# Entscheider/depthhead

Measured on AMD Instinct MI355X. Metric: depth frames/sec (640x480, 10-tree forest), higher is better.
Workload: dtype u32/f64

## Files before the change

### depthhead_amd/csrc/dh_api.hip

```cpp
#include "dh_runtime.h"
#include "dh_render.h"
#include "dh_runtime_track.h"

extern "C" const char *dh_last_error(void) { return dh_err_get_(); }
extern "C" int dh_version(void) { return DH_VERSION; }

static int forest_create_(const dh_forest_desc *d, dh_forest **out) { return dh_forest_build_(d, out); }

static int forest_destroy_(dh_forest *f) {
    delete f;
    return DH_OK;
}

static int forest_info_(const dh_forest *f, uint32_t *n_trees, uint32_t *n_nodes, uint32_t *n_leaves, uint32_t *max_depth) {
    if (!f) return fail(DH_EINVAL, "dh_forest_info: NULL forest");
    if (n_trees) *n_trees = (uint32_t)f->roots.size();
    if (n_nodes) *n_nodes = (uint32_t)f->nodes.size();
    if (n_leaves) *n_leaves = (uint32_t)f->leaf_prob.size();
    if (max_depth) *max_depth = f->max_depth;
    return DH_OK;
}

static int patch_grid_(const dh_params *p, int w, int h, int *nx, int *ny) {
    if (!p || !nx || !ny) return fail(DH_EINVAL, "dh_patch_grid: NULL argument");
// ... 538 lines not shown
    BoxArgs ba{};
    ba.frames = L.q.frames; ba.zeros = L.p->zeros.get(); ba.n_frames = L.n; ba.w = L.w; ba.h = L.h; ba.rw = L.p->f_rw; ba.rh = L.p->f_rh;
    ba.tile_flags = L.tile_flags; ba.tiles_x = g.tiles_x; ba.tiles_y = g.tiles_y; ba.gen = L.gen; ba.tpx = L.tpx; ba.tpy = L.tpy; ba.tbw = L.tw; ba.tbh = L.th;
    if (L.o.zero_fold) { ba.zero_ptr = ws.counters.get(); ba.zero_lo = (uint32_t)ws.lay.zero_lo; ba.zero_hi = (uint32_t)ws.lay.zero_hi; ba.zero_end = (uint32_t)ws.lay.zero_words; }
    ba.out = L.box; ba.plane = g.box_plane; ba.rows = g.box_rows; ba.lg = g.swz_log2; ba.ow = g.box_ow; ba.parts = g.box_parts;
    ba.ring = L.bp.ring; ba.oh = L.bp.oh; ba.bands = L.bp.bands; ba.blocks_per_frame = L.bp.blocks_per_frame;
    ba.blk_shift = ws.blk_shift; ba.mask_blocks = L.bp.mask_blocks; ba.blk_mask = L.blk_mask;
    if (L.use_list && ws.shifts.on) ba.list_count = L.tl_count;
    { Range r(L.o.profile, "dh:boxsum"); HIP_TRY(dh_launch_boxsum(ba, L.s)); }
    return DH_OK;
}
static int enqueue_tile_list(const Launch &L) {
    const Workspace &ws = L.ws; const Geom &g = L.g;
    Range r(L.o.profile, "dh:tile_list");
    if (!ws.shifts.on) { HIP_TRY(dh_launch_tile_list(L.tile_flags, L.gen, L.n, g.tiles_x * g.tiles_y, L.tl_list, L.tl_count, (uint32_t)ws.tile_list_stride, L.s)); return DH_OK; }
    TileShiftArgs sa{};
    sa.n_frames = L.n; sa.blk_shift = ws.blk_shift; sa.mask_blocks = L.bp.mask_blocks; sa.parts = g.box_parts; sa.blk_mask = L.blk_mask; sa.ow4 = g.box_ow / 4; sa.nc = g.box_parts * sa.ow4;
    sa.tiles_x = g.tiles_x; sa.tiles_y = g.tiles_y; sa.step = L.step; sa.tpx = L.tpx; sa.tpy = L.tpy; sa.tbw = L.tw; sa.tbh = L.th;
    sa.sx0 = ws.shifts.sx0; sa.sy0 = ws.shifts.sy0; sa.gx = ws.shifts.gx; sa.nsx = ws.shifts.nsx; sa.nsy = ws.shifts.nsy;
    sa.list = L.tl_list; sa.count = L.tl_count; sa.stride = (uint32_t)ws.tile_list_stride; sa.shift_out = ws.tile_shift.get() + L.f0;
    HIP_TRY(dh_launch_tile_shift(sa, L.s));
    return DH_OK;
}
static int enqueue_traverse(const Launch &L, bool *gated) {
    dh_predictor *p = L.p;
    const Workspace &ws = L.ws; const Geom &g = L.g;
    TraverseArgs ta{};
    ta.frames = L.q.frames; ta.n_frames = L.n; ta.w = L.w; ta.h = L.h;
    ta.step = L.step; ta.sw = (int)p->params.subimage_width; ta.sh = (int)p->params.subimage_height;
    ta.nx = g.nx; ta.ny = g.ny; ta.px = g.px; ta.py = g.py; ta.tiles_x = g.tiles_x; ta.tiles_y = g.tiles_y;
    ta.ss_max = g.ss_max; ta.ss_row = g.ss_row; ta.swz_log2 = g.swz_log2; ta.swz_q = g.swz_q;
    ta.uniform = g.uniform ? 1 : 0; ta.rw = p->f_rw; ta.rh = p->f_rh; ta.area = (uint32_t)(p->f_rw * p->f_rh);
    ta.nodes_u = p->nodes_u.get(); ta.nodes_a = p->absorb_ok ? p->nodes_a.get() : nullptr; ta.walk_lb = (p->n_nodes + p->n_amb) << 4; ta.amb_list = p->amb_list.get();
    ta.top_tab = p->top_tab.get(); ta.top_levels = g.top_levels; ta.nodes_g = p->knobs.no_general_int ? nullptr : p->nodes_g.get();
    ta.box = L.box; ta.box_plane = g.box_plane; ta.box_rows = g.box_rows; ta.tile_flags = L.tile_flags; ta.gen = L.gen;
#ifdef DH_PROFILING_KNOBS
    ta.stop_phase = p->knobs.trav_stop;
    if (p->knobs.trav_stamps)
        TRY(next_stamps(p->trav_stamps, 8, &ta.dbg_stamps, [](const unsigned long long *hst) {
            fprintf(stderr, "[k_traverse cycles/phase summed over the workgroups that reach it] region=%llu gate=%llu walks=%llu gated tail=%llu\n", hst[0], hst[1], hst[2], hst[3]);
        }));
#endif
    ta.f = p->dev; set_windows(ta, ws, L.f0, p->n_trees);
    *gated = !L.o.traverse_only && !L.o.leaf_out && !L.o.flags_out && dh_tile_gate_(g, ws.cap_frames, p->absorb_ok, p->n_trees, p->debug, p->knobs);
    if (*gated) { ta.tile_gate = 1; ta.win_total = ws.win_total(L.f0); }
    if (!L.o.traverse_only) p->ws.last_gated = *gated;
    ta.dbg_flags = L.dbg_flags; ta.dbg_leaf = L.o.leaf_out ? L.o.leaf_out : p->debug ? ws.dbg_leaf.get() + (size_t)L.f0 * g.npatch * p->n_trees : nullptr;
    if (L.use_list) { ta.tile_list = L.tl_list; ta.tile_list_count = L.tl_count; ta.tile_list_stride = (uint32_t)ws.tile_list_stride; }
    { Range r(L.o.profile, "dh:traverse"); HIP_TRY(dh_launch_traverse(ta, g.lds, L.s)); }
    return DH_OK;
}
static int enqueue_emit(const Launch &L, bool gated) {
    const Geom &g = L.g;
    EmitArgs ea{};
    ea.frames = L.q.frames; ea.n_frames = L.n; ea.w = L.w; ea.h = L.h;
    ea.step = L.step; ea.lw = L.lw; ea.lh = L.lh; ea.nx = g.nx; ea.npatch = g.npatch; ea.px = g.px; ea.py = g.py; ea.tiles = g.tiles_x * g.tiles_y;
    memcpy(ea.kinv, L.kinv, sizeof ea.kinv);
    ea.cams = L.cams; ea.f = L.p->dev; set_windows(ea, L.ws, L.f0, L.p->n_trees);
    if (gated) { ea.pre_gated = 1; ea.win_total = L.ws.win_total(L.f0); }
    set_hits(ea, L.ws, L.f0);
    ea.leaf_hits = L.q.heads ? nullptr : L.leaf_hits;
    ea.gen = L.gen; ea.dbg_flags = L.dbg_flags;
    if (L.q.support || L.q.heads) ea.hit_win = L.ws.hit_win.get() + L.hoff;
#ifdef DH_PROFILING_KNOBS
    ea.stop = L.p->knobs.emit_stop;
#endif
    { Range r(L.o.profile, "dh:emit"); HIP_TRY(dh_launch_emit(ea, L.s)); }
    return DH_OK;
}
static int enqueue_vote(const Launch &L) {
    const CamSel &cs = L.q.cams;
    VoteArgs va{};
    va.n_frames = L.n; va.w = L.w; va.h = L.h;
    va.cell_fast = !L.p->knobs.vote_exact && (!cs.c || cs.all_cell_fast(L.n, L.w, L.h)) ? 1 : 0;
    memcpy(va.k, L.K, sizeof va.k);
    va.cams = L.cams; va.cams_pin = cs.c && cs.all_pin(L.n) ? 1 : 0; va.f = L.p->dev;
    set_hits(va, L.ws, L.f0);
    va.pos_grid = L.pos_grid; va.rot_grid = L.rot_grid; va.leaf_hits = L.q.heads ? nullptr : L.leaf_hits;
#ifdef DH_PROFILING_KNOBS
    va.stop = L.p->knobs.vote_stop;
#endif
    { Range r(L.o.profile, "dh:vote"); HIP_TRY(dh_launch_vote(va, L.s)); }
    return DH_OK;
}
static ClusterArgs cluster_args(const Launch &L) {
    ClusterArgs ca{};
    ca.frames = L.q.frames; ca.n_frames = L.n; ca.w = L.w; ca.h = L.h;
    memcpy(ca.kinv, L.kinv, sizeof ca.kinv);
    ca.cams = L.cams; ca.f = L.p->dev; set_hits(ca, L.ws, L.f0);
    ca.pos_grid = L.pos_grid; ca.kern_r2 = L.p->kern_r2.get(); ca.iterations = L.p->params.meanshift_iterations;
    return ca;
}
static int enqueue_cluster(const Launch &L) {
    dh_predictor *p = L.p; const Workspace &ws = L.ws;
    ClusterArgs ca = cluster_args(L);
// ... 50 lines not shown
    SupportArgs sa{};
    sa.n_frames = L.n; sa.nx = L.g.nx; sa.step = L.step; sa.lw = L.lw; sa.lh = L.lh;
    sa.radius = L.q.radius; sa.poses = L.q.out; sa.out = L.q.support;
    sa.hits = ws.hits.get() + L.hoff; sa.hit_box = ws.hit_box.get() + L.hoff; sa.hit_win = ws.hit_win.get() + L.hoff;
    sa.hit_count = L.hit_count; sa.hits_cap = ws.hits_cap; sa.off4 = L.p->dev.off4;
    sa.acc = ws.sup_acc.get() + L.f0; sa.bits = ws.sup_bits.get() + (size_t)L.f0 * ws.sup_words; sa.bit_words = ws.sup_words;
    { Range r(L.o.profile, "dh:support"); HIP_TRY(dh_launch_support(sa, L.s)); }
    return DH_OK;
}

static int enqueue_range(dh_predictor *p, const BatchReq &sl, int f0, int n, hipStream_t s, const EnqueueOpts &o) {
    Launch L{p, sl.at(f0), f0, n, s, o};
    if (L.q.cams.c) memcpy(L.kinv, L.q.cams.c->host[L.q.cams.c0].kinv, sizeof L.kinv);
    else dh_mat3_inv_f32_(L.K, L.kinv);
    if (L.use_list) p->ws.list_chunks = std::max(p->ws.list_chunks, o.chunk + 1);
    const bool windows = L.g.npatch > 0;
    char batch_name[48];
    snprintf(batch_name, sizeof batch_name, "dh:batch n=%d %dx%d", n, L.w, L.h);
    Range batch_range(o.profile, batch_name);
    if (o.profile) HIP_TRY(hipEventRecord(p->ev[0], s));
    if (windows) TRY(enqueue_flags(L));
    if (L.use_list) TRY(enqueue_tile_list(L));
    if (o.profile) HIP_TRY(hipEventRecord(p->ev[4], s));
    bool gated = false;
    if (windows) TRY(enqueue_traverse(L, &gated));
    if (o.profile) HIP_TRY(hipEventRecord(p->ev[5], s));
    if (windows && !o.traverse_only) TRY(enqueue_emit(L, gated));
    if (o.profile) HIP_TRY(hipEventRecord(p->ev[1], s));
    if (o.traverse_only) return DH_OK;
    TRY(enqueue_vote(L));
    if (o.profile) HIP_TRY(hipEventRecord(p->ev[2], s));
    if (L.q.heads) TRY(enqueue_heads(L));
    else {
        TRY(enqueue_cluster(L));
        if (L.q.support) TRY(enqueue_support(L));
    }
    if (o.profile) { HIP_TRY(hipEventRecord(p->ev[3], s)); p->ev_valid = true; }
    return DH_OK;
}

static int max_resident_frames(const dh_predictor *p) { return p->knobs.max_resident; }

static int support_reserve(dh_predictor *p) {
    Workspace &ws = p->ws;
    if (ws.sup) return DH_OK;
    const size_t cap = (size_t)ws.cap_frames;
    ws.sup_words = (uint32_t)((std::max(ws.geom.npatch, 1) + 31) / 32);
    TRY(ws.hit_win.alloc(cap * ws.hits_cap));
    TRY(ws.sup_acc.alloc(cap));
    TRY(ws.sup_bits.alloc(cap * ws.sup_words));
    TRY(ws.sup.alloc(cap));
    if (hipMemsetAsync(ws.sup_acc.get(), 0, cap * sizeof(SupAcc), p->own_stream) != hipSuccess ||
        hipMemsetAsync(ws.sup_bits.get(), 0, cap * ws.sup_words * sizeof(uint32_t), p->own_stream) != hipSuccess ||
// ... 1011 lines not shown
        const Workspace &ws = p->ws;
        const Geom &g = ws.geom;
        const size_t bytes = (size_t)p->last_n * 4;
        if (g.npatch <= 0) { memset(out, 0, bytes); return DH_OK; }
        if (ws.last_gated) { HIP_TRY(hipMemcpy(out, ws.win_total(0), bytes, hipMemcpyDeviceToHost)); return DH_OK; }
        Buf<uint32_t> tot;
        TRY(tot.alloc(p->last_n));
        HIP_TRY(hipMemset(tot.get(), 0, bytes));
        EmitArgs ea{};
        ea.n_frames = p->last_n; ea.px = g.px; ea.py = g.py; ea.tiles = g.tiles_x * g.tiles_y; ea.f = p->dev;
        set_windows(ea, ws, 0, p->n_trees);
        HIP_TRY(dh_launch_window_totals(ea, tot.get(), nullptr));
        HIP_TRY(hipDeviceSynchronize());
        HIP_TRY(hipMemcpy(out, tot.get(), bytes, hipMemcpyDeviceToHost));
        return DH_OK;
    });
}
static int debug_geometry_(dh_predictor *p, int32_t out[10]) {
    if (!p || !out) return fail(DH_EINVAL, "NULL argument");
    if (p->ws.cap_frames == 0) return fail(DH_ESTATE, "no workspace yet (dh_predictor_reserve or a batch)");
    const Geom &g = p->ws.geom;
    const bool walk_tab = g.uniform && p->absorb_ok;
    const bool tile_gate = dh_tile_gate_(g, p->ws.cap_frames, p->absorb_ok, p->n_trees, p->debug, p->knobs);
    const int32_t v[10] = {(g.uniform ? 1 : 0) | (walk_tab ? 1 << 8 : 0) | (tile_gate ? 1 << 9 : 0) | (walk_tab ? g.top_levels << 16 : 0), g.px, g.py, g.tiles_x, g.tiles_y, g.swz_log2, g.swz_q, g.ss_row, p->f_rw, p->f_rh};
    memcpy(out, v, sizeof v);
    return DH_OK;
}
static int debug_tile_shifts_(dh_predictor *p, int32_t *shifts, uint32_t counts[8]) {
    return with_taps(p, false, [&]() -> int {
        const Workspace &ws = p->ws;
        if (!shifts || !counts) return fail(DH_EINVAL, "NULL output");
        if (ws.list_chunks == 0) return fail(DH_ESTATE, "the last batch ran without tile lists");
        std::vector<uint32_t> sh((size_t)p->last_n, 0u);
        if (ws.tile_shift) HIP_TRY(hipMemcpy(sh.data(), ws.tile_shift.get(), sh.size() * 4, hipMemcpyDeviceToHost));
        for (int f = 0; f < p->last_n; ++f) { shifts[2 * f] = (int32_t)(sh[f] & 0xffffu); shifts[2 * f + 1] = (int32_t)(sh[f] >> 16); }
        for (int x = 0; x < 8; ++x) counts[x] = 0;
        for (int c = 0; c < ws.list_chunks; ++c) {
            uint32_t cc[8];
            HIP_TRY(hipMemcpy(cc, ws.list_ptr(c) + 16 * ws.tile_list_stride, sizeof cc, hipMemcpyDeviceToHost));
            for (int x = 0; x < 8; ++x) counts[x] += cc[x];
        }
        return DH_OK;
    });
}
static int debug_guesses_(dh_predictor *p, int32_t *out) {
    return with_taps(p, true, [&]() -> int {
        if (!out) return fail(DH_EINVAL, "NULL output");
// ... 126 lines not shown
```

### depthhead_amd/csrc/dh_host.cpp

```cpp
#include "dh_host.h"

#include <limits.h>
#include <math.h>
#include <stdarg.h>
#include <stdio.h>
#include <stdlib.h>
#include <string.h>

#include <algorithm>
#include <cmath>
#include <atomic>
#include <string>
#include <thread>
#include <utility>

static thread_local char g_err[512] = "";

int dh_fail_(int code, const char *fmt, ...) {
    va_list ap;
    va_start(ap, fmt);
    vsnprintf(g_err, sizeof g_err, fmt, ap);
    va_end(ap);
    return code;
}
// ... 139 lines not shown
}

Knobs dh_read_knobs_() {
    Knobs k;
    auto geti = [](const char *name, int dflt) { const char *e = getenv(name); return e ? atoi(e) : dflt; };
    k.force_general = getenv("DH_FORCE_GENERAL") != nullptr;
    k.no_leaf_hist = getenv("DH_NO_LEAF_HIST") != nullptr;
    k.box_no_ring = getenv("DH_BOX_NO_RING") != nullptr;
    k.leaf_hist_max = (uint32_t)std::max(0, geti("DH_LEAF_HIST_MAX", 16384));
    k.lds_budget_kb = std::max(0, geti("DH_LDS_BUDGET_KB", 0));
    if (const char *e = getenv("DH_TILE")) {
        if (sscanf(e, "%d,%d", &k.tile_x, &k.tile_y) != 2 || k.tile_x < 1 || k.tile_y < 1) k.tile_x = k.tile_y = 0;
    }
    k.box_band = std::max(1, geti("DH_BOX_BAND", 64));
    k.box_bands = std::max(0, geti("DH_BOX_BANDS", 0));
    k.max_resident = std::max(1, geti("DH_MAX_RESIDENT_FRAMES", 512));
    k.chunks = std::max(0, std::min(8, geti("DH_CHUNKS", 0)));
    k.box_dense = getenv("DH_BOX_DENSE") != nullptr;
    k.no_region = getenv("DH_NO_REGION") != nullptr;
    k.region_min_hits = std::max(0, geti("DH_REGION_MIN_HITS", 0));
    k.no_general_int = getenv("DH_NO_GENERAL_INT") != nullptr;
    k.no_absorb = getenv("DH_NO_ABSORB") != nullptr;
    k.no_tile_gate = getenv("DH_NO_TILE_GATE") != nullptr;
    k.vote_exact = getenv("DH_VOTE_EXACT") != nullptr;
    k.no_tile_list = getenv("DH_NO_TILE_LIST") != nullptr;
    k.no_zero_fold = getenv("DH_NO_ZERO_FOLD") != nullptr;
    if (const char *e = getenv("DH_TILE_SHIFT")) {
        char tail = 0;
        if (strcmp(e, "off") == 0) k.tile_shift_mode = 1;
        else if (sscanf(e, "%d,%d%c", &k.tile_shift_x, &k.tile_shift_y, &tail) == 2 && k.tile_shift_x >= 0 && k.tile_shift_y >= 0) k.tile_shift_mode = 2;
        else k.tile_shift_mode = 3;
    }
    if (const char *e = getenv("DH_TOP_LEVELS")) k.top_levels = std::max(0, std::min(8, atoi(e)));
    k.stage_chunk = std::max(1, geti("DH_STAGE_CHUNK", 64));
    k.host_threads = std::max(1, std::min(64, geti("DH_HOST_THREADS", (int)std::max(1u, std::min(8u, std::thread::hardware_concurrency())))));
#ifdef DH_PROFILING_KNOBS
    k.trav_stop = geti("DH_TRAV_STOP", 0); k.emit_stop = geti("DH_EMIT_STOP", 0);
    k.vote_stop = geti("DH_VOTE_STOP", 0); k.cl_stop = geti("DH_CL_STOP", 0);
    k.trav_stamps = getenv("DH_TRAV_STAMPS") != nullptr;
    k.cl_stamps = getenv("DH_CL_STAMPS") != nullptr;
#endif
    return k;
}

int dh_patch_grid_(const dh_params &p, int w, int h, int *nx, int *ny) {
    if (p.stepwidth == 0 || p.subimage_width == 0 || p.subimage_height == 0) return dh_fail_(DH_EINVAL, "zero stepwidth / patch size");
// ... 336 lines not shown
```

### depthhead_amd/csrc/dh_host.h

```cpp
#pragma once
#include <stddef.h>
#include <stdint.h>

#include <functional>
#include <new>
#include <vector>

#include "../../include/depthhead_hip.h"

int dh_fail_(int code, const char *fmt, ...) __attribute__((format(printf, 2, 3)));
const char *dh_err_get_(void);
void dh_err_set_(const char *msg);

template <typename F>
static inline int dh_guard_(const char *what, F &&body) noexcept {
    try {
        return body();
    } catch (const std::bad_alloc &) {
        return dh_fail_(DH_ENOMEM, "%s: out of host memory", what);
    } catch (const std::exception &e) {
        return dh_fail_(DH_EINVAL, "%s: %s", what, e.what());
    } catch (...) {
        return dh_fail_(DH_EINVAL, "%s: unexpected exception", what);
    }
// ... 27 lines not shown

struct Knobs {
    bool force_general = false;
    bool no_leaf_hist = false;
    bool box_no_ring = false;
    uint32_t leaf_hist_max = 16384;
    int lds_budget_kb = 0;
    int tile_x = 0, tile_y = 0;
    int box_band = 64;
    int box_bands = 0;
    int max_resident = 512;
    int chunks = 0;
    bool box_dense = false;
    bool no_region = false;
    int region_min_hits = 0;
    int top_levels = -1;
    bool no_zero_fold = false;
    bool no_tile_list = false;
    int tile_shift_mode = 0;
    int tile_shift_x = 0, tile_shift_y = 0;
    bool vote_exact = false;
    bool no_absorb = false;
    bool no_tile_gate = false;
    bool no_general_int = false;
    int stage_chunk = 64;
    int host_threads = 8;
    bool cl_stamps = false;
    int trav_stop = 0, emit_stop = 0, vote_stop = 0, cl_stop = 0;
    bool trav_stamps = false;
};
Knobs dh_read_knobs_();

struct Geom {
    int w = 0, h = 0, nx = 0, ny = 0, npatch = 0;
    int px = 0, py = 0, tiles_x = 0, tiles_y = 0, ss_max = 0, ss_row = 0, swz_log2 = 0, swz_q = 0;
    bool uniform = false;
    int top_levels = 0;
    int flag_words = 0;
    int win_cap = 0;
    int box_plane = 0, box_rows = 0, box_ow = 0, box_oh = 0, box_parts = 0, box_bands = 0;
    size_t lds = 0;
};
int dh_patch_grid_(const dh_params &p, int w, int h, int *nx, int *ny);

void dh_traverse_swizzle(int px, int step, int sw, int rw, int *swz_log2, int *swz_q, int *ss_row);
int dh_traverse_row_stride(int px, int step, int sw, int rw);
// ... 8 lines not shown
    bool one_pass = false;
    int lds_budget_kb = 0, tile_x = 0, tile_y = 0, box_band = 64;
};
int dh_choose_tile_(const TileQuery &q, Geom &g);
struct TileShifts {
    bool on = false;
    int gx = 1, nsx = 1, nsy = 1, sx0 = 0, sy0 = 0;
};
#define DH_TILE_SHIFT_LDS_WORDS 12288
static inline size_t dh_tile_shift_lds_words(int mask_blocks, int parts, int nc, int n_shifts) {
    return (size_t)2 * mask_blocks * parts + (size_t)(mask_blocks + 1) * (nc + 1) + (size_t)n_shifts + 8;
}
int dh_tile_shifts_(const Geom &g, int step, int blk_shift, const Knobs &k, TileShifts *out);
static const int kBoxSpan = 256, kBoxMaxRect = 96;
int dh_box_bands_(int n, int parts, int rows, int blk, int rh, int wg_slots, int *oh);
static inline int dh_mask_blocks_(int rows, int blk_shift) { return (rows + (1 << blk_shift) - 1) >> blk_shift; }
struct BoxPlan { int ring = 0, oh = 0, bands = 0, mask_blocks = 0, blocks_per_frame = 0; };
__attribute__((visibility("hidden"))) BoxPlan dh_box_plan_(int n, const Geom &g, int rh, int blk_shift, const Knobs &k);
static inline bool dh_use_tile_list_(bool has_lists, int npatch, bool outputs_or_taps, int n, int tiles) {
    return has_lists && npatch > 0 && !outputs_or_taps && (long)n * tiles > 512;
}

bool dh_tile_gate_(const Geom &g, int cap_frames, bool absorb_ok, uint32_t n_trees, bool taps, const Knobs &k);

#define DH_GRID3 8000
#define DH_POSGRID 400
struct CounterLayout {
    size_t tiles = 0, leaves = 0;
    size_t hit_count = 0, pos_grid = 0, rot_grid = 0, tile_flags = 0, win_count = 0, leaf_hits = 0;
    size_t zero_lo = 0, zero_hi = 0;
    size_t zero_words = 0;
    size_t alloc_words = 0;
};
CounterLayout dh_counter_layout_(size_t cap, size_t flag_words, size_t tiles, size_t leaf_hist_leaves);

void dh_mat3_inv_f32_(const float m[9], float o[9]);
void dh_build_kernel_r2_(float sigma, std::vector<float> &k, size_t padded);
void dh_build_kernel_table_(float sigma, std::vector<float> &k);
int dh_blur_taps_(float sigma, std::vector<float> &k);

bool dh_vote_cell_fast_(const float K[9], int w, int h);

#define DH_STAGE_EVENTS 16
int dh_chunk_plan_(int m, int stage_chunk, bool single, int cstart[DH_STAGE_EVENTS + 1]);

struct DhRun { uint32_t dst, src; };
// ... 11 lines not shown
```

### depthhead_amd/csrc/dh_internal.h

```cpp
#pragma once
#include <hip/hip_runtime.h>
#include <stddef.h>
#include <stdint.h>

#include "dh_host.h"
#include "dh_train.h"

#define DH_GRID 20
#define DH_ROTPARTS 120
#define DH_REGION_CELLS (26 * 26 * 26)
#define DH_KERN_R2 304
#define DH_SUPER_CELLS (64 * 64 * 64)

#define LF_PROB 1u
#define LF_ROT 2u
#define LF_OFF 4u
#define LF_FIN 8u

struct __attribute__((aligned(16))) DhCam {
    float k[9];
    float kinv[9];
    uint32_t pin;
    uint32_t pad;
};
// ... 71 lines not shown
    int box_plane, box_rows;
    const uint2 *tile_list;
    const uint32_t *tile_list_count;
    uint32_t tile_list_stride;
    const uint32_t *gen;
    const uint8_t *tile_flags;
    const void *nodes_u;
    const void *nodes_a;
    uint32_t walk_lb;
    const uint32_t *amb_list;
    const uint32_t *top_tab;
    int top_levels;
    const void *nodes_g;
    unsigned long long *dbg_stamps;
    int stop_phase;
    DevForest f;
    uint32_t *win_count;
    uint32_t *win_patch;
    void     *win_leaf;
    int       leaf_ls;
    int       win_cap;
    uint32_t *win_total;
    int       tile_gate;
    int32_t  *dbg_leaf;
    uint8_t  *dbg_flags;
};

struct EmitArgs {
    const uint16_t *frames;
    int n_frames, w, h;
    int step, lw, lh;
    int nx, npatch;
    int px, py, tiles;
    float kinv[9];
    DevForest f;
    const uint32_t *win_count;
    const uint32_t *win_patch;
    const void     *win_leaf;
    int       leaf_ls;
    int       win_cap;
    const uint32_t *win_total;
    int       pre_gated;
    HitRec   *hits;
    HitBox   *hit_box;
    HitRot   *hit_rot;
    uint32_t *hit_count;
// ... 50 lines not shown
    const uint32_t *gen;
    int tiles_x, tiles_y;
    int tpx, tpy, tfw, tfh;
};

struct VoteArgs {
    int n_frames, w, h;
    float k[9];
    DevForest f;
    const HitRec   *hits;
    const HitBox   *hit_box;
    const HitRot   *hit_rot;
    const uint32_t *hit_count;
    uint32_t  hits_cap;
    uint32_t *pos_grid;
    uint32_t *rot_grid;
    const uint32_t *leaf_hits;
    int stop;
    int cell_fast;
    float sx, sy;
    float kxs, cxs, kys, cys;
    const DhCam *cams;
    int cams_pin;
};

struct ClusterArgs {
    const uint16_t *frames;
    int n_frames, w, h;
    float kinv[9];
    DevForest f;
    const HitRec   *hits;
    const HitBox   *hit_box;
    const HitRot   *hit_rot;
    const uint32_t *hit_count;
    uint32_t  hits_cap;
    const uint32_t *leaf_hits;
    const uint32_t *pos_grid;
    const uint32_t *rot_grid;
    const float    *kern_r2;
    uint32_t  iterations;
    const float   *midp_guess;
    const double  *rot_guess;
    const uint8_t *guess_mask;
    dh_pose  *out;
    uint32_t *pre_region;
    int       pre_slices;
// ... 234 lines not shown
```

### depthhead_amd/csrc/k_traverse.hip

```cpp
#include "dh_device.h"

#ifndef TRAV_THREADS
#define TRAV_THREADS 1024
#endif
#define TRAV_WMAX (4096 / TRAV_THREADS)
#define TRAV_WAVES (TRAV_THREADS / WAVE)
#define ROWS_IN_FLIGHT 8

template <int PPL>
__device__ __forceinline__ bool sat_rows_dpp(uint32_t *sat, uint32_t *flag, const uint16_t *img, int w, int fx0, int fy0,
                                             int fw, int fh, int ss) {
    constexpr int RMAX = 16 / PPL;
    const int tid = threadIdx.x, lane = tid & (WAVE - 1), wave = tid >> 6;
    const int R = (fh + TRAV_WAVES - 1) / TRAV_WAVES;
    const int y0 = wave * R, x0 = lane * PPL;
    const bool al = ((w % PPL) == 0) && ((fx0 % PPL) == 0) && ((((size_t)img) & (PPL * 2 - 1)) == 0);
    uint32_t p[RMAX][PPL];
    uint32_t any_px = 0;
    const uint16_t *org = img + (size_t)fy0 * w + fx0;
    if (al) {
        const bool fullx = x0 + PPL <= fw;
        uint32_t raw[RMAX][PPL / 2];
#pragma unroll
        for (int r = 0; r < RMAX; ++r) {
// ... 411 lines not shown
                if (cur[i] >= 0) cur[i] = one ? (int)n1[i].y : (int)n1[i].x;
            }
        }
#pragma unroll
        for (int i = 0; i < W; ++i)
            if (k0 + i * TRAV_THREADS < total) {
                store_leaf(wleaf, a.leaf_ls, dst[i], ~cur[i]);
                if (dleaf) dleaf[ddst[i]] = ~cur[i];
            }
    }
}

#ifdef DH_PROFILING_KNOBS
#define STAMP(k)                                                                        \
    if (a.dbg_stamps && tid == 0) {                                                     \
        unsigned long long t_ = clock64();                                              \
        atomicAdd(&a.dbg_stamps[k], t_ - t_prev);                                        \
        t_prev = t_;                                                                    \
    }
#else
#define STAMP(k)
#endif

template <bool UNI, bool GI, bool GATE = false>
__global__ void __launch_bounds__(TRAV_THREADS, TRAV_THREADS / 128) k_traverse(TraverseArgs a) {
    extern __shared__ __attribute__((aligned(16))) uint32_t lds[];
    const int tid = threadIdx.x, lane = tid & (WAVE - 1);
    const int T = (int)a.f.n_trees;

    int frame = (int)blockIdx.z * 8 + (int)blockIdx.x;
    int tile = (int)blockIdx.y;
    int sx = 0, sy = 0;
    if (a.tile_list) {
        const uint32_t k = blockIdx.y + gridDim.y * blockIdx.z;
        const uint2 e = a.tile_list[(size_t)blockIdx.x * a.tile_list_stride + k];
        const uint32_t cnt = a.tile_list_count[blockIdx.x];
        if (k >= cnt) return;
        frame = (int)(e.x >> 16) * 8 + (int)blockIdx.x; tile = (int)(e.x & 0xffffu);
        sx = (int)(e.y & 0xffffu); sy = (int)(e.y >> 16);
    }
    if (frame >= a.n_frames || KNOB_STOP(a.stop_phase == 9)) return;
    const int ty = div_small(tile, a.tiles_x, 1.0f / (float)a.tiles_x), tx = tile - ty * a.tiles_x;
    const int wx0 = max(0, tx * a.px - sx), wy0 = max(0, ty * a.py - sy);
    const int cx = min(a.nx, (tx + 1) * a.px - sx) - wx0, cy = min(a.ny, (ty + 1) * a.py - sy) - wy0;
    const float r_cx = 1.0f / (float)cx;
    const int npt = cx * cy;
    const int fx0 = wx0 * a.step, fy0 = wy0 * a.step;
// ... 177 lines not shown

    STAMP(2)

    if (GATE) {
        if (KNOB_STOP(a.stop_phase == 4)) return;
        __syncthreads();
        double *pprob = (double *)sat;
#pragma unroll
        for (int i = 0; i < TRAV_WMAX; ++i) {
            const int k = tid + i * TRAV_THREADS;
            if (k < total) pprob[k] = gpr[i];
        }
        __syncthreads();
        if (__builtin_amdgcn_readfirstlane(tid & ~(WAVE - 1)) < n_active) {
            bool gated = false;
            if (tid < n_active) {
                double prob = 0.0;
                for (int t = 0; t < T; ++t) prob = __dadd_rn(prob, pprob[t * n_active + tid]);
                prob = __ddiv_rn(prob, (double)T);
                gated = prob > DH_PROB_GATE;
            }
            const unsigned long long bal = __ballot(gated);
            uint32_t lslot = 0xffffffffu;
            if (bal) {
                uint32_t wave_base = 0;
                if (lane == 0) wave_base = atomicAdd(&a.win_total[frame], (uint32_t)__popcll(bal));
                wave_base = __shfl(wave_base, 0);
                if (gated) lslot = wave_base + (uint32_t)__popcll(bal & ((1ull << lane) - 1ull));
                if (lslot < (uint32_t)a.win_cap) a.win_patch[(size_t)frame * a.win_cap + lslot] = agp[tid];
            }
            if (tid < n_active) active[tid] = lslot;
        }
        __syncthreads();
        char *fl = (char *)a.win_leaf + (((size_t)frame * a.win_cap * T) << a.leaf_ls);
        const float r_act = 1.0f / (float)n_active;
#pragma unroll
        for (int i = 0; i < TRAV_WMAX; ++i) {
            const int k = tid + i * TRAV_THREADS;
            if (k < total) {
                const int t = div_small(k, n_active, r_act);
                const uint32_t lslot = active[k - t * n_active];
                if (lslot < (uint32_t)a.win_cap) store_leaf(fl, a.leaf_ls, t * a.win_cap + (int)lslot, (int32_t)gl[i]);
            }
        }
        STAMP(3)
    }
}

#include <algorithm>
#include <atomic>
hipError_t dh_kernels_init(int device) {
    static std::atomic<unsigned long long> done[4];
    const bool tracked = device >= 0 && device < 256;
    if (tracked && (done[device >> 6].load(std::memory_order_acquire) >> (device & 63)) & 1ull) return hipSuccess;
    hipError_t e = hipFuncSetAttribute((const void *)k_traverse<true, false>, hipFuncAttributeMaxDynamicSharedMemorySize, 160 * 1024);
    if (e == hipSuccess) e = hipFuncSetAttribute((const void *)k_traverse<true, true>, hipFuncAttributeMaxDynamicSharedMemorySize, 160 * 1024);
    if (e == hipSuccess) e = hipFuncSetAttribute((const void *)k_traverse<true, true, true>, hipFuncAttributeMaxDynamicSharedMemorySize, 160 * 1024);
    if (e == hipSuccess) e = hipFuncSetAttribute((const void *)k_traverse<false, false>, hipFuncAttributeMaxDynamicSharedMemorySize, 160 * 1024);
    if (e == hipSuccess) e = hipFuncSetAttribute((const void *)k_traverse<false, true>, hipFuncAttributeMaxDynamicSharedMemorySize, 160 * 1024);
    if (e == hipSuccess) e = dh_region_init();
    if (e != hipSuccess) return e;
    if (tracked) done[device >> 6].fetch_or(1ull << (device & 63), std::memory_order_release);
    return hipSuccess;
}

hipError_t dh_launch_traverse(const TraverseArgs &a, size_t lds_bytes, hipStream_t s) {
    const int tiles = a.tiles_x * a.tiles_y, fb = (a.n_frames + 7) / 8;
    if (tiles == 0 || fb == 0) return hipSuccess;
    if (tiles > 65535 || fb > 65535) return hipErrorInvalidConfiguration;
    const dim3 grid((unsigned)std::min(8, a.n_frames), tiles, fb);
    if (a.tile_gate && !(a.uniform && a.nodes_a && a.win_total)) return hipErrorInvalidValue;
    if (a.tile_gate) hipLaunchKernelGGL((k_traverse<true, true, true>), grid, dim3(TRAV_THREADS), lds_bytes, s, a);
    else if (a.uniform && a.nodes_a) hipLaunchKernelGGL((k_traverse<true, true>), grid, dim3(TRAV_THREADS), lds_bytes, s, a);
    else if (a.uniform) hipLaunchKernelGGL((k_traverse<true, false>), grid, dim3(TRAV_THREADS), lds_bytes, s, a);
    else if (a.nodes_g) hipLaunchKernelGGL((k_traverse<false, true>), grid, dim3(TRAV_THREADS), lds_bytes, s, a);
    else hipLaunchKernelGGL((k_traverse<false, false>), grid, dim3(TRAV_THREADS), lds_bytes, s, a);
    return hipGetLastError();
}
```

### depthhead_amd/csrc/k_vote.hip

```cpp
#include "dh_device.h"

#define VOTE_THREADS 512
#ifndef VOTE_SLICES
#define VOTE_SLICES 8
#endif
#define VOTE_TAB 2048
#ifndef VOTE_SUB
#define VOTE_SUB 4u
#endif
#ifndef VOTE_ILP
#define VOTE_ILP 12
#endif

template <bool TAB, bool PINNED>
__device__ __forceinline__ void vote_positions(const VoteArgs &a, uint32_t *pos, const uint8_t *gxt, const uint8_t *gyt, const float4 rec,
                                               uint32_t v, uint32_t fc, uint32_t sub, float wm1, float hm1) {
    const uint32_t ob = __float_as_uint(rec.w), oe = ob + (fc >> 8);
    uint32_t last = 0xFFFFFFFFu, acc = 0;
    for (uint32_t o0 = ob + sub; o0 < oe; o0 += VOTE_SUB * VOTE_ILP) {
        float ox[VOTE_ILP], oy[VOTE_ILP], oz[VOTE_ILP];
#pragma unroll
        for (int j = 0; j < VOTE_ILP; ++j) {
            const uint32_t o = min(o0 + VOTE_SUB * j, oe - 1);
            const float4 of = a.f.off4[o];
// ... 34 lines not shown
                const uint32_t xi = (uint32_t)x2, yi = (uint32_t)y2;
                const uint32_t gx = TAB ? gxt[xi] : xi * DH_GRID / (uint32_t)a.w;
                const uint32_t gy = TAB ? gyt[yi] : yi * DH_GRID / (uint32_t)a.h;
                idx = gy * DH_GRID + gx;
            }
            if (idx != last) {
                if (acc) atomicAdd(&pos[last], acc);
                last = idx; acc = 0;
            }
            acc += v;
        }
    }
    if (acc) atomicAdd(&pos[last], acc);
}

__device__ __forceinline__ float sgpr_f32(float x) { return __int_as_float(__builtin_amdgcn_readfirstlane(__float_as_int(x))); }

template <bool TAB, bool PIN, bool LH, bool CAM>
__global__ void __launch_bounds__(VOTE_THREADS) k_vote(VoteArgs a) {
    __shared__ uint32_t pos[DH_POSGRID];
    __shared__ uint32_t rot[DH_GRID3];
    __shared__ uint8_t gxt[VOTE_TAB], gyt[VOTE_TAB];
    const int frame = blockIdx.y, tid = threadIdx.x;
    if (CAM) {
        const DhCam *c = a.cams + frame;
#pragma unroll
        for (int i = 0; i < 9; ++i) a.k[i] = c->k[i];
        a.kxs = sgpr_f32(__fmul_rn(a.k[0], a.sx)); a.cxs = sgpr_f32(__fmul_rn(a.k[2], a.sx));
        a.kys = sgpr_f32(__fmul_rn(a.k[4], a.sy)); a.cys = sgpr_f32(__fmul_rn(a.k[5], a.sy));
    }
    uint32_t n = a.hit_count[frame];
    if (n > a.hits_cap) n = a.hits_cap;
    const uint32_t slices = gridDim.x;
    const uint32_t per = (n + slices - 1) / slices;
    const uint32_t h0 = min(n, blockIdx.x * per), h1 = min(n, h0 + per);
    if (n == 0 || (h0 >= h1 && !LH)) return;
    for (int i = tid; i < DH_POSGRID; i += VOTE_THREADS) pos[i] = 0;
    for (int i = tid; i < DH_GRID3; i += VOTE_THREADS) rot[i] = 0;
    if (TAB) {
        for (int i = tid; i < a.w; i += VOTE_THREADS) gxt[i] = (uint8_t)((uint32_t)i * DH_GRID / (uint32_t)a.w);
        for (int i = tid; i < a.h; i += VOTE_THREADS) gyt[i] = (uint8_t)((uint32_t)i * DH_GRID / (uint32_t)a.h);
    }
    __syncthreads();
    if (KNOB_STOP(a.stop == 1)) return;
    const HitRec *hits = a.hits + (size_t)frame * a.hits_cap;
    const HitBox *box = a.hit_box + (size_t)frame * a.hits_cap;
// ... 73 lines not shown
```

### depthhead_amd/prediction.py

```python
from __future__ import annotations

import ctypes as C
from dataclasses import dataclass

import numpy as np

from . import _lib
from ._lib import HEAD_DTYPE, MAX_HEADS, POSE_DTYPE, SUPPORT_DTYPE, SUPPORT_RADIUS, check, vp
from .forest import Forest
from .synth import ModelParams


def _host_frames(img):
    frames = np.ascontiguousarray(img, dtype=np.uint16)
    single = frames.ndim == 2
    if single:
        frames = frames[None]
    n, h, w = frames.shape
    return frames, single, n, h, w


def _batch_frames(frames):
    frames = np.ascontiguousarray(frames, dtype=np.uint16)
    if frames.ndim != 3:
# ... 308 lines not shown
    def debug_patch_flags(self, n: int, w: int, h: int) -> np.ndarray:
        nx, ny = self.patch_grid(w, h)
        out = np.zeros((n, nx * ny), dtype=np.uint8)
        check(self._lib.dh_debug_patch_flags(self._ph, vp(out), C.c_size_t(out.size)))
        return out

    def debug_grids(self, n: int):
        pos = np.zeros((n, 400), dtype=np.uint32)
        rot = np.zeros((n, 8000), dtype=np.uint32)
        check(self._lib.dh_debug_grids(self._ph, vp(pos), vp(rot)))
        return pos, rot

    def debug_guesses(self, n: int) -> np.ndarray:
        out = np.zeros((n, 6), dtype=np.int32)
        check(self._lib.dh_debug_guesses(self._ph, vp(out)))
        return out

    def debug_geometry(self) -> dict:
        out = np.zeros(10, dtype=np.int32)
        check(self._lib.dh_debug_geometry(self._ph, vp(out)))
        keys = ("uniform", "px", "py", "tiles_x", "tiles_y", "swz_log2", "swz_q", "ss_row", "rw", "rh")
        geo = dict(zip(keys, (int(x) for x in out)))
        path = geo["uniform"]
        geo.update(uniform=path & 1, walk_table=(path >> 8) & 1, tile_gate=bool((path >> 9) & 1), top_levels=path >> 16)
        return geo

    def debug_tile_shifts(self, n: int) -> tuple[np.ndarray, np.ndarray]:
        shifts, counts = np.zeros((n, 2), dtype=np.int32), np.zeros(8, dtype=np.uint32)
        check(self._lib.dh_debug_tile_shifts(self._ph, vp(shifts), vp(counts)))
        return shifts, counts

    def debug_hit_counts(self, n: int) -> np.ndarray:
        out = np.zeros(n, dtype=np.uint32)
        check(self._lib.dh_debug_hit_counts(self._ph, vp(out)))
        return out

    def debug_window_totals(self, n: int) -> np.ndarray:
        out = np.zeros(n, dtype=np.uint32)
        check(self._lib.dh_debug_window_totals(self._ph, vp(out)))
        return out

    def debug_votes(self, frame: int, which: int, cap: int = 1 << 22) -> np.ndarray:
        out = np.zeros((cap, 4), dtype=np.int32)
        cnt = C.c_size_t()
        check(self._lib.dh_debug_votes(self._ph, C.c_int(frame), C.c_int(which), vp(out), C.c_size_t(cap), C.byref(cnt)))
        if cnt.value > cap:
            return self.debug_votes(frame, which, int(cnt.value))
# ... 24 lines not shown
```

Before: 778,300.

## Fuse hit emission into gated traverse kernel, skipping separate emit launch

When tile gating is active, the traverse kernel now builds the vote hit records itself instead of writing leaf indices to window buffers for a separate emit kernel. Each workgroup compacts voting leaves into shared memory, reserves hit slots with one atomic, and writes positions, boxes, rotations and leaf-hit histograms directly. The emit launch is skipped and the generation counter bump moves into the vote kernel. This removes the intermediate window-leaf write/read and a kernel launch, but adds register and LDS pressure and tail work to the traverse kernel.

```diff
diff --git a/depthhead_amd/csrc/dh_api.hip b/depthhead_amd/csrc/dh_api.hip
--- a/depthhead_amd/csrc/dh_api.hip
+++ b/depthhead_amd/csrc/dh_api.hip
@@ -584,7 +584,7 @@
     HIP_TRY(dh_launch_tile_shift(sa, L.s));
     return DH_OK;
 }
-static int enqueue_traverse(const Launch &L, bool *gated) {
+static int enqueue_traverse(const Launch &L, bool *gated, bool *emitted) {
     dh_predictor *p = L.p;
     const Workspace &ws = L.ws; const Geom &g = L.g;
     TraverseArgs ta{};
@@ -600,13 +600,21 @@
     ta.stop_phase = p->knobs.trav_stop;
     if (p->knobs.trav_stamps)
         TRY(next_stamps(p->trav_stamps, 8, &ta.dbg_stamps, [](const unsigned long long *hst) {
-            fprintf(stderr, "[k_traverse cycles/phase summed over the workgroups that reach it] region=%llu gate=%llu walks=%llu gated tail=%llu\n", hst[0], hst[1], hst[2], hst[3]);
+            fprintf(stderr, "[k_traverse cycles/phase summed over the workgroups that reach it] region=%llu gate=%llu walks=%llu gated tail=%llu record step=%llu | tiles in the tail=%llu, of them in the record step=%llu\n",
+                    hst[0], hst[1], hst[2], hst[3], hst[4], hst[6], hst[7]);
         }));
 #endif
     ta.f = p->dev; set_windows(ta, ws, L.f0, p->n_trees);
     *gated = !L.o.traverse_only && !L.o.leaf_out && !L.o.flags_out && dh_tile_gate_(g, ws.cap_frames, p->absorb_ok, p->n_trees, p->debug, p->knobs);
     if (*gated) { ta.tile_gate = 1; ta.win_total = ws.win_total(L.f0); }
     if (!L.o.traverse_only) p->ws.last_gated = *gated;
+    *emitted = dh_tile_emit_(*gated, L.dbg_flags != nullptr, p->knobs);
+    if (*emitted) {
+        ta.tile_emit = 1; ta.lw = L.lw; ta.lh = L.lh; memcpy(ta.kinv, L.kinv, sizeof ta.kinv); ta.cams = L.cams;
+        set_hits(ta, ws, L.f0);
+        ta.leaf_hits = L.q.heads ? nullptr : L.leaf_hits;
+        if (L.q.support || L.q.heads) ta.hit_win = ws.hit_win.get() + L.hoff;
+    }
     ta.dbg_flags = L.dbg_flags; ta.dbg_leaf = L.o.leaf_out ? L.o.leaf_out : p->debug ? ws.dbg_leaf.get() + (size_t)L.f0 * g.npatch * p->n_trees : nullptr;
     if (L.use_list) { ta.tile_list = L.tl_list; ta.tile_list_count = L.tl_count; ta.tile_list_stride = (uint32_t)ws.tile_list_stride; }
     { Range r(L.o.profile, "dh:traverse"); HIP_TRY(dh_launch_traverse(ta, g.lds, L.s)); }
@@ -630,9 +638,10 @@
     { Range r(L.o.profile, "dh:emit"); HIP_TRY(dh_launch_emit(ea, L.s)); }
     return DH_OK;
 }
-static int enqueue_vote(const Launch &L) {
+static int enqueue_vote(const Launch &L, bool emitted) {
     const CamSel &cs = L.q.cams;
     VoteArgs va{};
+    if (emitted) va.gen = L.gen;
     va.n_frames = L.n; va.w = L.w; va.h = L.h;
     va.cell_fast = !L.p->knobs.vote_exact && (!cs.c || cs.all_cell_fast(L.n, L.w, L.h)) ? 1 : 0;
     memcpy(va.k, L.K, sizeof va.k);
@@ -729,13 +738,13 @@
     if (windows) TRY(enqueue_flags(L));
     if (L.use_list) TRY(enqueue_tile_list(L));
     if (o.profile) HIP_TRY(hipEventRecord(p->ev[4], s));
-    bool gated = false;
-    if (windows) TRY(enqueue_traverse(L, &gated));
+    bool gated = false, emitted = false;
+    if (windows) TRY(enqueue_traverse(L, &gated, &emitted));
     if (o.profile) HIP_TRY(hipEventRecord(p->ev[5], s));
-    if (windows && !o.traverse_only) TRY(enqueue_emit(L, gated));
+    if (windows && !o.traverse_only && !emitted) TRY(enqueue_emit(L, gated));
     if (o.profile) HIP_TRY(hipEventRecord(p->ev[1], s));
     if (o.traverse_only) return DH_OK;
-    TRY(enqueue_vote(L));
+    TRY(enqueue_vote(L, emitted));
     if (o.profile) HIP_TRY(hipEventRecord(p->ev[2], s));
     if (L.q.heads) TRY(enqueue_heads(L));
     else {
@@ -1793,7 +1802,8 @@
     const Geom &g = p->ws.geom;
     const bool walk_tab = g.uniform && p->absorb_ok;
     const bool tile_gate = dh_tile_gate_(g, p->ws.cap_frames, p->absorb_ok, p->n_trees, p->debug, p->knobs);
-    const int32_t v[10] = {(g.uniform ? 1 : 0) | (walk_tab ? 1 << 8 : 0) | (tile_gate ? 1 << 9 : 0) | (walk_tab ? g.top_levels << 16 : 0), g.px, g.py, g.tiles_x, g.tiles_y, g.swz_log2, g.swz_q, g.ss_row, p->f_rw, p->f_rh};
+    const bool tile_emit = dh_tile_emit_(tile_gate, p->debug, p->knobs);
+    const int32_t v[10] = {(g.uniform ? 1 : 0) | (walk_tab ? 1 << 8 : 0) | (tile_gate ? 1 << 9 : 0) | (tile_emit ? 1 << 10 : 0) | (walk_tab ? g.top_levels << 16 : 0), g.px, g.py, g.tiles_x, g.tiles_y, g.swz_log2, g.swz_q, g.ss_row, p->f_rw, p->f_rh};
     memcpy(out, v, sizeof v);
     return DH_OK;
 }
diff --git a/depthhead_amd/csrc/dh_host.cpp b/depthhead_amd/csrc/dh_host.cpp
--- a/depthhead_amd/csrc/dh_host.cpp
+++ b/depthhead_amd/csrc/dh_host.cpp
@@ -185,6 +185,7 @@
     k.no_general_int = getenv("DH_NO_GENERAL_INT") != nullptr;
     k.no_absorb = getenv("DH_NO_ABSORB") != nullptr;
     k.no_tile_gate = getenv("DH_NO_TILE_GATE") != nullptr;
+    k.no_tile_emit = getenv("DH_NO_TILE_EMIT") != nullptr;
     k.vote_exact = getenv("DH_VOTE_EXACT") != nullptr;
     k.no_tile_list = getenv("DH_NO_TILE_LIST") != nullptr;
     k.no_zero_fold = getenv("DH_NO_ZERO_FOLD") != nullptr;
diff --git a/depthhead_amd/csrc/dh_host.h b/depthhead_amd/csrc/dh_host.h
--- a/depthhead_amd/csrc/dh_host.h
+++ b/depthhead_amd/csrc/dh_host.h
@@ -73,6 +73,7 @@
     bool vote_exact = false;
     bool no_absorb = false;
     bool no_tile_gate = false;
+    bool no_tile_emit = false;
     bool no_general_int = false;
     int stage_chunk = 64;
     int host_threads = 8;
@@ -127,6 +128,7 @@
 }
 
 bool dh_tile_gate_(const Geom &g, int cap_frames, bool absorb_ok, uint32_t n_trees, bool taps, const Knobs &k);
+static inline bool dh_tile_emit_(bool tile_gate, bool taps, const Knobs &k) { return tile_gate && !taps && !k.no_tile_emit; }
 
 #define DH_GRID3 8000
 #define DH_POSGRID 400
diff --git a/depthhead_amd/csrc/dh_internal.h b/depthhead_amd/csrc/dh_internal.h
--- a/depthhead_amd/csrc/dh_internal.h
+++ b/depthhead_amd/csrc/dh_internal.h
@@ -117,6 +117,17 @@
     int       win_cap;
     uint32_t *win_total;
     int       tile_gate;
+    int       tile_emit;
+    int       lw, lh;
+    float     kinv[9];
+    const DhCam *cams;
+    HitRec   *hits;
+    HitBox   *hit_box;
+    HitRot   *hit_rot;
+    uint32_t *hit_count;
+    uint32_t  hits_cap;
+    uint32_t *leaf_hits;
+    uint32_t *hit_win;
     int32_t  *dbg_leaf;
     uint8_t  *dbg_flags;
 };
@@ -213,6 +224,7 @@
     float kxs, cxs, kys, cys;
     const DhCam *cams;
     int cams_pin;
+    uint32_t *gen;
 };
 
 struct ClusterArgs {
diff --git a/depthhead_amd/csrc/k_traverse.hip b/depthhead_amd/csrc/k_traverse.hip
--- a/depthhead_amd/csrc/k_traverse.hip
+++ b/depthhead_amd/csrc/k_traverse.hip
@@ -457,7 +457,7 @@
 #define STAMP(k)
 #endif
 
-template <bool UNI, bool GI, bool GATE = false>
+template <bool UNI, bool GI, bool GATE = false, bool EMIT = false>
 __global__ void __launch_bounds__(TRAV_THREADS, TRAV_THREADS / 128) k_traverse(TraverseArgs a) {
     extern __shared__ __attribute__((aligned(16))) uint32_t lds[];
     const int tid = threadIdx.x, lane = tid & (WAVE - 1);
@@ -681,6 +681,10 @@
             }
             const unsigned long long bal = __ballot(gated);
             uint32_t lslot = 0xffffffffu;
+            if (EMIT) {
+                if (bal && lane == 0) { atomicAdd(&a.win_total[frame], (uint32_t)__popcll(bal)); misc[5] = 1u; }
+                if (gated) lslot = 0u;
+            } else
             if (bal) {
                 uint32_t wave_base = 0;
                 if (lane == 0) wave_base = atomicAdd(&a.win_total[frame], (uint32_t)__popcll(bal));
@@ -691,18 +695,115 @@
             if (tid < n_active) active[tid] = lslot;
         }
         __syncthreads();
-        char *fl = (char *)a.win_leaf + (((size_t)frame * a.win_cap * T) << a.leaf_ls);
         const float r_act = 1.0f / (float)n_active;
+        if (!EMIT) {
+            char *fl = (char *)a.win_leaf + (((size_t)frame * a.win_cap * T) << a.leaf_ls);
+#pragma unroll
+            for (int i = 0; i < TRAV_WMAX; ++i) {
+                const int k = tid + i * TRAV_THREADS;
+                if (k < total) {
+                    const int t = div_small(k, n_active, r_act);
+                    const uint32_t lslot = active[k - t * n_active];
+                    if (lslot < (uint32_t)a.win_cap) store_leaf(fl, a.leaf_ls, t * a.win_cap + (int)lslot, (int32_t)gl[i]);
+                }
+            }
+            STAMP(3)
+            return;
+        }
+        STAMP(3)
+#ifdef DH_PROFILING_KNOBS
+        if (a.dbg_stamps && tid == 0) atomicAdd(&a.dbg_stamps[6], 1ull);
+#endif
+        if (misc[5] == 0u || KNOB_STOP(a.stop_phase == 5)) return;
+#ifdef DH_PROFILING_KNOBS
+        if (a.dbg_stamps && tid == 0) atomicAdd(&a.dbg_stamps[7], 1ull);
+#endif
+        uint2 *rlist = (uint2 *)sat;
+        uint32_t votes = 0;
+        uint32_t before[TRAV_WMAX], wave_n = 0;
 #pragma unroll
         for (int i = 0; i < TRAV_WMAX; ++i) {
             const int k = tid + i * TRAV_THREADS;
+            bool v = false;
             if (k < total) {
                 const int t = div_small(k, n_active, r_act);
-                const uint32_t lslot = active[k - t * n_active];
-                if (lslot < (uint32_t)a.win_cap) store_leaf(fl, a.leaf_ls, t * a.win_cap + (int)lslot, (int32_t)gl[i]);
-            }
-        }
-        STAMP(3)
+                if (active[k - t * n_active] == 0u) {
+                    const uint32_t lf = a.f.leaf_flags[gl[i]];
+                    v = (lf & LF_PROB) && (lf & (LF_ROT | LF_OFF));
+                }
+            }
+            const unsigned long long bal = __ballot(v);
+            before[i] = wave_n + (uint32_t)__popcll(bal & ((1ull << lane) - 1ull));
+            wave_n += (uint32_t)__popcll(bal);
+            if (v) votes |= 1u << i;
+        }
+        uint32_t wave_base = 0;
+        if (wave_n && lane == 0) wave_base = atomicAdd(&misc[6], wave_n);
+        wave_base = __shfl(wave_base, 0);
+#pragma unroll
+        for (int i = 0; i < TRAV_WMAX; ++i)
+            if ((votes >> i) & 1u) {
+                const int k = tid + i * TRAV_THREADS;
+                const int t = div_small(k, n_active, r_act);
+                rlist[wave_base + before[i]] = make_uint2(gl[i], agp[k - t * n_active]);
+            }
+        __syncthreads();
+        const uint32_t nrec = misc[6];
+        if (nrec == 0u) return;
+        if (tid == 0) misc[7] = atomicAdd(&a.hit_count[frame], nrec);
+        float kinv[9];
+        if (a.cams) cam_kinv(kinv, a.cams + __builtin_amdgcn_readfirstlane(frame));
+        else {
+#pragma unroll
+            for (int i = 0; i < 9; ++i) kinv[i] = a.kinv[i];
+        }
+        HitRec *dst = a.hits + (size_t)frame * a.hits_cap;
+        HitBox *dbox = a.hit_box + (size_t)frame * a.hits_cap;
+        HitRot *drot = a.hit_rot + (size_t)frame * a.hits_cap;
+        uint32_t base = 0;
+#pragma unroll 1
+        for (uint32_t r0 = 0; r0 < nrec; r0 += TRAV_THREADS) {
+            const uint32_t r = r0 + (uint32_t)tid;
+            const bool has = r < nrec;
+            const uint2 e = rlist[has ? r : 0u];
+            const uint32_t lid = e.x, gp = e.y;
+            const uint4 *tp = (const uint4 *)(a.f.tpl + lid);
+            const uint4 t0 = tp[0], t1 = tp[1], t2v = tp[2], t3 = tp[3];
+            const int gyi = (int)(gp / (uint32_t)a.nx), gxi = (int)gp - gyi * a.nx;
+            const uint16_t zc = img[(size_t)(gyi * a.step + a.lh) * a.w + gxi * a.step + a.lw];
+            if (r0 == 0u) { __syncthreads(); base = misc[7]; }
+            const uint32_t o = base + r;
+            if (has && o < a.hits_cap) {
+                float q[3];
+                to3d(kinv, (float)(gxi * a.step + a.lw), (float)(gyi * a.step + a.lh), (float)zc, q);
+                const float p0 = q[0], p1 = q[1], p2 = q[2];
+                const float mn0 = __uint_as_float(t0.x), mn1 = __uint_as_float(t0.y), mn2 = __uint_as_float(t0.z),
+                            mx0 = __uint_as_float(t0.w), mx1 = __uint_as_float(t1.x), mx2 = __uint_as_float(t1.y);
+                *(float4 *)(dst + o) = make_float4(p0, p1, p2, __uint_as_float(t2v.x));
+                ((int4 *)(dbox + o))[0] = make_int4(f32_as_i32(__fsub_rn(p0, mx0)), f32_as_i32(__fsub_rn(p1, mx1)),
+                                                     f32_as_i32(__fsub_rn(p2, mx2)), f32_as_i32(__fsub_rn(p0, mn0)));
+                ((int4 *)(dbox + o))[1] = make_int4(f32_as_i32(__fsub_rn(p1, mn1)), f32_as_i32(__fsub_rn(p2, mn2)), (int)t1.z, (int)t1.w);
+                if (!a.leaf_hits || a.dbg_flags) *(uint4 *)(drot + o) = make_uint4(t2v.y, t2v.z, t2v.w, t3.x);
+#ifdef TRAV_EXP_PLAIN_HIST
+                if (a.leaf_hits && (t1.w & LF_ROT)) atomicAdd(&a.leaf_hits[(size_t)frame * a.f.n_leaves + lid], 1u);
+#endif
+                if (a.hit_win) a.hit_win[(size_t)frame * a.hits_cap + o] = gp;
+            }
+#if !defined(TRAV_EXP_PLAIN_HIST) && !defined(TRAV_EXP_NO_HIST)
+            if (a.leaf_hits) {
+                const bool v = has && o < a.hits_cap && (t1.w & LF_ROT);
+                const uint32_t key = v ? lid : 0xFFFFFFFFu;
+                const uint32_t prev = (uint32_t)__shfl_up((int)key, 1);
+                const bool cont = v && lane > 0 && prev == key;
+                const unsigned long long c = __ballot(cont);
+                if (v && !cont) {
+                    const unsigned long long rest = lane == WAVE - 1 ? 0ull : (c >> (lane + 1));
+                    atomicAdd(&a.leaf_hits[(size_t)frame * a.f.n_leaves + key], 1u + (uint32_t)__builtin_ctzll(~rest));
+                }
+            }
+#endif
+        }
+        STAMP(4)
     }
 }
 
@@ -715,6 +816,7 @@
     hipError_t e = hipFuncSetAttribute((const void *)k_traverse<true, false>, hipFuncAttributeMaxDynamicSharedMemorySize, 160 * 1024);
     if (e == hipSuccess) e = hipFuncSetAttribute((const void *)k_traverse<true, true>, hipFuncAttributeMaxDynamicSharedMemorySize, 160 * 1024);
     if (e == hipSuccess) e = hipFuncSetAttribute((const void *)k_traverse<true, true, true>, hipFuncAttributeMaxDynamicSharedMemorySize, 160 * 1024);
+    if (e == hipSuccess) e = hipFuncSetAttribute((const void *)k_traverse<true, true, true, true>, hipFuncAttributeMaxDynamicSharedMemorySize, 160 * 1024);
     if (e == hipSuccess) e = hipFuncSetAttribute((const void *)k_traverse<false, false>, hipFuncAttributeMaxDynamicSharedMemorySize, 160 * 1024);
     if (e == hipSuccess) e = hipFuncSetAttribute((const void *)k_traverse<false, true>, hipFuncAttributeMaxDynamicSharedMemorySize, 160 * 1024);
     if (e == hipSuccess) e = dh_region_init();
@@ -729,7 +831,9 @@
     if (tiles > 65535 || fb > 65535) return hipErrorInvalidConfiguration;
     const dim3 grid((unsigned)std::min(8, a.n_frames), tiles, fb);
     if (a.tile_gate && !(a.uniform && a.nodes_a && a.win_total)) return hipErrorInvalidValue;
-    if (a.tile_gate) hipLaunchKernelGGL((k_traverse<true, true, true>), grid, dim3(TRAV_THREADS), lds_bytes, s, a);
+    if (a.tile_emit && !(a.tile_gate && a.hits && a.hit_box && a.hit_rot && a.hit_count)) return hipErrorInvalidValue;
+    if (a.tile_emit) hipLaunchKernelGGL((k_traverse<true, true, true, true>), grid, dim3(TRAV_THREADS), lds_bytes, s, a);
+    else if (a.tile_gate) hipLaunchKernelGGL((k_traverse<true, true, true>), grid, dim3(TRAV_THREADS), lds_bytes, s, a);
     else if (a.uniform && a.nodes_a) hipLaunchKernelGGL((k_traverse<true, true>), grid, dim3(TRAV_THREADS), lds_bytes, s, a);
     else if (a.uniform) hipLaunchKernelGGL((k_traverse<true, false>), grid, dim3(TRAV_THREADS), lds_bytes, s, a);
     else if (a.nodes_g) hipLaunchKernelGGL((k_traverse<false, true>), grid, dim3(TRAV_THREADS), lds_bytes, s, a);
diff --git a/depthhead_amd/csrc/k_vote.hip b/depthhead_amd/csrc/k_vote.hip
--- a/depthhead_amd/csrc/k_vote.hip
+++ b/depthhead_amd/csrc/k_vote.hip
@@ -80,6 +80,7 @@
     __shared__ uint32_t rot[DH_GRID3];
     __shared__ uint8_t gxt[VOTE_TAB], gyt[VOTE_TAB];
     const int frame = blockIdx.y, tid = threadIdx.x;
+    if (a.gen && blockIdx.x == 0 && blockIdx.y == 0 && tid == 0) *a.gen = *a.gen % 255u + 1u;
     if (CAM) {
         const DhCam *c = a.cams + frame;
 #pragma unroll
diff --git a/depthhead_amd/prediction.py b/depthhead_amd/prediction.py
--- a/depthhead_amd/prediction.py
+++ b/depthhead_amd/prediction.py
@@ -354,7 +354,8 @@
         keys = ("uniform", "px", "py", "tiles_x", "tiles_y", "swz_log2", "swz_q", "ss_row", "rw", "rh")
         geo = dict(zip(keys, (int(x) for x in out)))
         path = geo["uniform"]
-        geo.update(uniform=path & 1, walk_table=(path >> 8) & 1, tile_gate=bool((path >> 9) & 1), top_levels=path >> 16)
+        geo.update(uniform=path & 1, walk_table=(path >> 8) & 1, tile_gate=bool((path >> 9) & 1), tile_emit=bool((path >> 10) & 1),
+                   top_levels=path >> 16)
         return geo
 
     def debug_tile_shifts(self, n: int) -> tuple[np.ndarray, np.ndarray]:
```

After: 769,800. 1.1% lower.
